# kkaitlyn111/cs336-a2-systems

Measured on AMD Instinct MI355X. Metric: tokens/sec/node GPT-2-XL bf16 DDP, higher is better.
Workload: dtype bf16; 1 GPU; global_batch=102, per_gpu_batch=102, seq_len=512, parallelism=dp1, ddp=none, optimizer=fused HIP AdamW (fp32 master weights), overlapped with backward, attention=HIP FlashAttention-2 (causal), hip_graph=False, gemm_selection=per-problem fastest of hipblaslt default / autotuned lt_gemm / cs336 MFMA GEMM

## Files before the change

### csrc/gemm/gemm8.h

```cpp
#pragma once

#include <hip/hip_runtime.h>
#include <stdint.h>

namespace cs336 {
namespace gemm8 {

struct Args {
  const uint16_t* a;
  const uint16_t* b;
  uint16_t* c;
  uint16_t* h;
  const uint16_t* y;
  int64_t lda, ldb, ldc, ldh, ldy;
  int M, N, K;
  int half;
  const float* rcos;
  const float* rsin;
  const int64_t* rpos;
  int rseq, rope_cols, rdh;
  uint64_t* stamps = nullptr;
};
int pick_fn(int N, int epi, int half);
bool set_stamp_buffer(uint64_t* buf, int64_t blocks);
bool launch(const Args& p, int epi, int fn, hipStream_t s);

struct WArgs {
  const uint16_t* a;
  const uint16_t* b;
  float* c;
  int64_t lda, ldb, ldc, slab_stride;
  int64_t a_elems, b_elems;
  int M, N, K;
  int splits;
  int trans_out, accumulate;
  uint64_t* stamps = nullptr;
  int64_t stamp_rows = 0;
};
bool launch_w(const WArgs& p, int fn, hipStream_t s);

}
}
```

### csrc/gemm/gemm8.hip

```cpp
#include "cs336/kernels.h"
#include "gemm8.h"

namespace cs336 {
namespace gemm8 {


namespace {

typedef __attribute__((ext_vector_type(8))) __bf16 bf16x8;
typedef __attribute__((ext_vector_type(4))) float f32x4;
typedef __attribute__((ext_vector_type(4))) unsigned int v4u32;
typedef __attribute__((address_space(3))) void* lds_ptr_t;

constexpr int BM = 256, BK = 64, NT = 512;
constexpr int kGroupM = 8;

__device__ __forceinline__ int xcd_remap(int bid, int total) {
  const int xcd = bid & 7, q = total >> 3, r = total & 7;
  const int base = xcd < r ? xcd * (q + 1) : r * (q + 1) + (xcd - r) * q;
  return base + (bid >> 3);
}

__device__ __forceinline__ void sbarrier() {
  __builtin_amdgcn_sched_barrier(0);
  asm volatile("s_barrier" ::: "memory");
  __builtin_amdgcn_sched_barrier(0);
}
__device__ __forceinline__ void lgkm0() { asm volatile("s_waitcnt lgkmcnt(0)" ::: "memory"); }
template <int N>
__device__ __forceinline__ void vmcnt() {
  asm volatile("s_waitcnt vmcnt(%0)" ::"n"(N) : "memory");
}

__device__ __forceinline__ float sigmoid_f(float a) { return __builtin_amdgcn_rcpf(1.f + __expf(-a)); }

template <int FN>
struct Geo {
  static constexpr int BN = 64 * FN;
  static constexpr int WTN = 16 * FN;
  static constexpr int FB0 = (FN + 1) / 2;
  static constexpr int B0C = 16 * FB0;
  static constexpr int A_BYTES = BM * 128;
  static constexpr int B_BYTES = BN * 128;
  static constexpr int STAGE = A_BYTES + B_BYTES;
  static constexpr int G_A0 = 16 / 8;
  static constexpr int G_B0 = (4 * B0C / 8) / 8;
  static constexpr int G_B1 = (4 * (WTN - B0C) / 8) / 8;
  static constexpr int G_A1 = 16 / 8;
  static constexpr int G_P1 = G_A0 + G_B0, G_P2 = G_B1, G_P3 = G_A1;
  static constexpr int G_ALL = G_P1 + G_P2 + G_P3;
  static_assert((4 * B0C / 8) % 8 == 0 && (4 * (WTN - B0C) / 8) % 8 == 0, "B granules must split over 8 waves");
};

template <int FN, int EPI, int TAIL>
__global__ __launch_bounds__(NT, 2) void gemm8_kernel(const Args p) {
  static_assert(!TAIL || EPI == 0, "tails: plain C = A·Bᵀ only");
  constexpr bool NTAIL = TAIL & 1, KTAIL = TAIL & 2;
  using G = Geo<FN>;
  constexpr int BN = G::BN, WTN = G::WTN, FB0 = G::FB0, B0C = G::B0C, STAGE = G::STAGE;
  __shared__ __attribute__((aligned(1024))) char smem[2 * STAGE > BM * BN * 2 ? 2 * STAGE : BM * BN * 2];

  const int tid = threadIdx.x, lane = tid & 63;
  const int wave = __builtin_amdgcn_readfirstlane(tid >> 6);
  const int wr = wave >> 2, wc = wave & 3;
#ifdef CS336_G8_STAMP
  const uint64_t st_t0 = __builtin_amdgcn_s_memtime(), st_r0 = __builtin_amdgcn_s_memrealtime();
  uint64_t st_t1 = 0, st_t2 = 0;
#endif

  const int tiles_n = NTAIL ? (p.N + BN - 1) / BN : p.N / BN;
  const int tiles_m = p.M / BM;
  const int bid = xcd_remap(blockIdx.x, gridDim.x);
  const int per_group = kGroupM * tiles_n;
  const int first_m = (bid / per_group) * kGroupM;
  const int gsz = min(tiles_m - first_m, kGroupM);
  const int tm = first_m + (bid % per_group) % gsz, tn = (bid % per_group) / gsz;
  const int m0 = tm * BM;
  const int n0 = tn * (EPI == 1 ? BN / 2 : BN);

  const int nkt = KTAIL ? (p.K + BK - 1) / BK : p.K / BK;
  constexpr uint32_t kOOB = 0x7ffffff0u;
  const __amdgpu_buffer_rsrc_t ra = __builtin_amdgcn_make_buffer_rsrc(
      (void*)(p.a + (int64_t)m0 * p.lda), (short)0, (uint32_t)(((BM - 1) * p.lda + p.K) * 2), 0x00020000);
  const __amdgpu_buffer_rsrc_t rb = __builtin_amdgcn_make_buffer_rsrc(
      (void*)p.b, (short)0, (uint32_t)(((int64_t)(p.N - 1) * p.ldb + p.K) * 2), 0x00020000);
  uint32_t voff[G::G_ALL];
  uint32_t ldso[G::G_ALL];
  {
    int s = 0;
    auto a_gran = [&](int row0) {
      const int r = row0 + (lane >> 3), lc = (lane & 7) ^ ((r >> 1) & 7);
      voff[s] = 2u * (uint32_t)(r * p.lda + lc * 8);
      ldso[s] = (uint32_t)(row0 * 128);
      ++s;
    };
    auto b_gran = [&](int row0) {
      const int r = row0 + (lane >> 3), lc = (lane & 7) ^ ((r >> 1) & 7);
      int grow;
      if constexpr (EPI == 1) grow = r < BN / 2 ? n0 + r : p.half + n0 + (r - BN / 2);
      else grow = n0 + r;
      voff[s] = 2u * (uint32_t)((int64_t)grow * p.ldb + lc * 8);
      ldso[s] = (uint32_t)(G::A_BYTES + row0 * 128);
      ++s;
    };
#pragma unroll
    for (int i = 0; i < G::G_A0; ++i) {
      const int g = wave + 8 * i;
      a_gran(g < 8 ? 8 * g : 128 + 8 * (g - 8));
    }
#pragma unroll
    for (int i = 0; i < G::G_B0; ++i) {
      const int g = wave + 8 * i, per = B0C / 8;
      b_gran((g / per) * WTN + (g % per) * 8);
    }
#pragma unroll
    for (int i = 0; i < G::G_B1; ++i) {
      const int g = wave + 8 * i, per = (WTN - B0C) / 8;
      b_gran((g / per) * WTN + B0C + (g % per) * 8);
    }
#pragma unroll
    for (int i = 0; i < G::G_A1; ++i) {
      const int g = wave + 8 * i;
      a_gran(g < 8 ? 64 + 8 * g : 192 + 8 * (g - 8));
    }
  }
  auto glds = [&](const __amdgpu_buffer_rsrc_t& rs, uint32_t vo, uint32_t so, uint32_t lds_off) {
    __builtin_amdgcn_raw_ptr_buffer_load_lds(rs, (lds_ptr_t)(smem + lds_off), 16, vo, so, 0, 0);
  };
  auto gran_row = [&](int i) -> int {
    if (i < G::G_A0) {
      const int g = wave + 8 * i;
      return g < 8 ? 8 * g : 128 + 8 * (g - 8);
    } else if (i < G::G_P1) {
      const int g = wave + 8 * (i - G::G_A0), per = B0C / 8;
      return (g / per) * WTN + (g % per) * 8;
    } else if (i < G::G_P1 + G::G_P2) {
      const int g = wave + 8 * (i - G::G_P1), per = (WTN - B0C) / 8;
      return (g / per) * WTN + B0C + (g % per) * 8;
    }
    const int g = wave + 8 * (i - G::G_P1 - G::G_P2);
    return g < 8 ? 64 + 8 * g : 192 + 8 * (g - 8);
  };
  auto issue_v = [&](int part, int kt, int st, bool masked) {
    const uint32_t so = (uint32_t)kt * (BK * 2), base = (uint32_t)(st * STAGE);
    auto vo = [&](int i) -> uint32_t {
      if (!masked) return voff[i];
      const int ln = __lane_id(), r = gran_row(i) + (ln >> 3), lc = (ln & 7) ^ ((r >> 1) & 7);
      return kt * BK + lc * 8 >= p.K ? kOOB : voff[i];
    };
    if (part == 0 || part == 1) {
#pragma unroll
      for (int i = 0; i < G::G_A0; ++i) glds(ra, vo(i), so, base + ldso[i]);
#pragma unroll
      for (int i = G::G_A0; i < G::G_P1; ++i) glds(rb, vo(i), so, base + ldso[i]);
    }
    if (part == 0 || part == 2) {
#pragma unroll
      for (int i = G::G_P1; i < G::G_P1 + G::G_P2; ++i) glds(rb, vo(i), so, base + ldso[i]);
    }
    if (part == 0 || part == 3) {
#pragma unroll
      for (int i = G::G_P1 + G::G_P2; i < G::G_ALL; ++i) glds(ra, vo(i), so, base + ldso[i]);
    }
  };
  auto issue = [&](int part, int kt, int st) {
    if (KTAIL && kt == nkt - 1) issue_v(part, kt, st, true);
    else issue_v(part, kt, st, false);
  };

  const int x = (lane & 15) >> 1, q4 = lane >> 4;
  const uint32_t lo0 = (uint32_t)((lane & 15) * 128 + ((q4 ^ x) * 16));
  const uint32_t lo1 = (uint32_t)((lane & 15) * 128 + (((4 + q4) ^ x) * 16));
  auto frag = [&](uint32_t img_off, int row0, int ks) -> bf16x8 {
    const char* ptr = smem + img_off + row0 * 128 + (ks ? lo1 : lo0);
    return __builtin_bit_cast(bf16x8, *reinterpret_cast<const uint4*>(ptr));
  };

  f32x4 acc[8][FN];
#pragma unroll
  for (int i = 0; i < 8; ++i)
#pragma unroll
    for (int j = 0; j < FN; ++j) acc[i][j] = f32x4{0.f, 0.f, 0.f, 0.f};

  bf16x8 fa[4][2], fb0[FB0][2], fb1[FN - FB0 > 0 ? FN - FB0 : 1][2];
  const int arow = wr * 128, bcol = wc * WTN;

  auto mma = [&](int i0, const bf16x8 (&a)[4][2], auto& bq, int j0, int nj) {
    __builtin_amdgcn_s_setprio(1);
#pragma unroll
    for (int ks = 0; ks < 2; ++ks)
#pragma unroll
      for (int i = 0; i < 4; ++i)
#pragma unroll
        for (int j = 0; j < nj; ++j)
          acc[i0 + i][j0 + j] = __builtin_amdgcn_mfma_f32_16x16x32_bf16(bq[j][ks], a[i][ks], acc[i0 + i][j0 + j], 0, 0, 0);
    __builtin_amdgcn_s_setprio(0);
  };

  issue(0, 0, 0);
  if (nkt > 1) {
    issue(0, 1, 1);
    vmcnt<G::G_ALL>();
  } else {
    vmcnt<0>();
  }
  sbarrier();
#ifdef CS336_G8_STAMP
  st_t1 = __builtin_amdgcn_s_memtime();
#endif
  if (wr == 1) sbarrier();

  for (int t = 0; t < nkt; ++t) {
    const uint32_t st = (uint32_t)((t & 1) * STAGE);
    const bool pre = t + 2 < nkt;
#pragma unroll
    for (int i = 0; i < 4; ++i)
#pragma unroll
      for (int ks = 0; ks < 2; ++ks) fa[i][ks] = frag(st, arow + 16 * i, ks);
#pragma unroll
    for (int j = 0; j < FB0; ++j)
#pragma unroll
      for (int ks = 0; ks < 2; ++ks) fb0[j][ks] = frag(st + G::A_BYTES, bcol + 16 * j, ks);
    lgkm0();
    sbarrier();
    mma(0, fa, fb0, 0, FB0);
    sbarrier();
    if constexpr (FN - FB0 > 0) {
#pragma unroll
      for (int j = 0; j < FN - FB0; ++j)
#pragma unroll
        for (int ks = 0; ks < 2; ++ks) fb1[j][ks] = frag(st + G::A_BYTES, bcol + B0C + 16 * j, ks);
    }
    if (pre) issue(1, t + 2, t & 1);
    lgkm0();
    sbarrier();
    if constexpr (FN - FB0 > 0) mma(0, fa, fb1, FB0, FN - FB0);
    sbarrier();
#pragma unroll
    for (int i = 0; i < 4; ++i)
#pragma unroll
      for (int ks = 0; ks < 2; ++ks) fa[i][ks] = frag(st, arow + 64 + 16 * i, ks);
    if (pre) issue(2, t + 2, t & 1);
    lgkm0();
    sbarrier();
    if constexpr (FN - FB0 > 0) mma(4, fa, fb1, FB0, FN - FB0);
    sbarrier();
    if (t + 1 < nkt) {
      if (pre) vmcnt<G::G_P1 + G::G_P2>();
      else vmcnt<0>();
    }
    if (pre) issue(3, t + 2, t & 1);
    sbarrier();
    mma(4, fa, fb0, 0, FB0);
    sbarrier();
  }
  if (wr == 0) sbarrier();
  lgkm0();
  sbarrier();
#ifdef CS336_G8_STAMP
  st_t2 = __builtin_amdgcn_s_memtime();
#endif

  constexpr int ST_AUX = EPI == 0 ? 0 : 2, LD_AUX = 2;
  const int m_l = lane & 15, n_l = 4 * (lane >> 4);
  if constexpr (EPI != 3) {
    constexpr int RB = BN * 2, CH = BN / 8;
    auto img = [&](int row, int ch) -> uint32_t {
      const int x = FN == 5 ? ((row >> 1) & 7) : (row & 15);
      return (uint32_t)(row * RB + ((ch ^ x) << 4));
    };
#pragma unroll
    for (int i = 0; i < 8; ++i)
#pragma unroll
      for (int j = 0; j < FN; ++j) {
        const f32x4 v = acc[i][j];
        const int row = arow + 16 * i + m_l, col = bcol + 16 * j + n_l;
        const uint32_t lo = (uint32_t)f32_to_bf16(v[0]) | ((uint32_t)f32_to_bf16(v[1]) << 16);
        const uint32_t hi = (uint32_t)f32_to_bf16(v[2]) | ((uint32_t)f32_to_bf16(v[3]) << 16);
        *reinterpret_cast<uint2*>(smem + img(row, col >> 3) + ((col >> 2) & 1) * 8) = make_uint2(lo, hi);
      }
    const __amdgpu_buffer_rsrc_t rc = __builtin_amdgcn_make_buffer_rsrc(
        (void*)(p.c + (int64_t)m0 * p.ldc), (short)0, 0x7fffffffu, 0x00020000);
    if constexpr (EPI == 2) {
      constexpr int PT = BM * CH / NT;
      static_assert(BM * CH % NT == 0, "chunks must split over the workgroup");
      const __amdgpu_buffer_rsrc_t ry = __builtin_amdgcn_make_buffer_rsrc(
          (void*)(p.y + (int64_t)m0 * p.ldy), (short)0, 0x7fffffffu, 0x00020000);
      uint4 av[PT], bv[PT];
#pragma unroll
      for (int i = 0; i < PT; ++i) {
        const int q = tid + NT * i, row = q / CH, ch = q % CH;
        const uint32_t off = 2u * (uint32_t)(row * p.ldy + n0 + 8 * ch);
        av[i] = __builtin_bit_cast(uint4, __builtin_amdgcn_raw_buffer_load_b128(ry, off, 0, LD_AUX));
        bv[i] = __builtin_bit_cast(uint4, __builtin_amdgcn_raw_buffer_load_b128(ry, off + 2u * (uint32_t)p.half, 0, LD_AUX));
      }
      lgkm0();
      sbarrier();
#pragma unroll
      for (int i = 0; i < PT; ++i) {
        const int q = tid + NT * i, row = q / CH, ch = q % CH;
        const uint4 dv = *reinterpret_cast<const uint4*>(smem + img(row, ch));
        const bf16_t* de = reinterpret_cast<const bf16_t*>(&dv);
        const bf16_t* ae = reinterpret_cast<const bf16_t*>(&av[i]);
        const bf16_t* be = reinterpret_cast<const bf16_t*>(&bv[i]);
        uint4 dav, dbv;
        bf16_t* da = reinterpret_cast<bf16_t*>(&dav);
        bf16_t* db = reinterpret_cast<bf16_t*>(&dbv);
#pragma unroll
        for (int e = 0; e < 8; ++e) {
          const float a = bf16_to_f32(ae[e]), b = bf16_to_f32(be[e]), dh = bf16_to_f32(de[e]);
          const float sg = sigmoid_f(a), gb = dh * sg;
          da[e] = f32_to_bf16(gb * b * (1.f + a * (1.f - sg)));
          db[e] = f32_to_bf16(gb * a);
        }
        const uint32_t off = 2u * (uint32_t)(row * p.ldc + n0 + 8 * ch);
        __builtin_amdgcn_raw_buffer_store_b128(__builtin_bit_cast(v4u32, dav), rc, off, 0, ST_AUX);
        __builtin_amdgcn_raw_buffer_store_b128(__builtin_bit_cast(v4u32, dbv), rc, off + 2u * (uint32_t)p.half, 0, ST_AUX);
      }
    } else if constexpr (EPI == 1) {
      constexpr int HU = CH / 2, PT = BM * HU / NT;
      static_assert(BM * HU % NT == 0, "pairs must split over the workgroup");
      const __amdgpu_buffer_rsrc_t rh = __builtin_amdgcn_make_buffer_rsrc(
          (void*)(p.h + (int64_t)m0 * p.ldh), (short)0, 0x7fffffffu, 0x00020000);
      lgkm0();
      sbarrier();
#pragma unroll
      for (int i = 0; i < PT; ++i) {
        const int q = tid + NT * i, row = q / HU, u = q % HU;
        const uint4 va = *reinterpret_cast<const uint4*>(smem + img(row, u));
        const uint4 vb = *reinterpret_cast<const uint4*>(smem + img(row, u + HU));
        const uint32_t off = 2u * (uint32_t)(row * p.ldc + n0 + 8 * u);
        __builtin_amdgcn_raw_buffer_store_b128(__builtin_bit_cast(v4u32, va), rc, off, 0, ST_AUX);
        __builtin_amdgcn_raw_buffer_store_b128(__builtin_bit_cast(v4u32, vb), rc, off + 2u * (uint32_t)p.half, 0, ST_AUX);
        const bf16_t* ae = reinterpret_cast<const bf16_t*>(&va);
        const bf16_t* be = reinterpret_cast<const bf16_t*>(&vb);
        uint4 hv;
        bf16_t* he = reinterpret_cast<bf16_t*>(&hv);
#pragma unroll
        for (int e = 0; e < 8; ++e) {
          const float a = bf16_to_f32(ae[e]);
          he[e] = f32_to_bf16(a * sigmoid_f(a) * bf16_to_f32(be[e]));
        }
        __builtin_amdgcn_raw_buffer_store_b128(__builtin_bit_cast(v4u32, hv), rh, 2u * (uint32_t)(row * p.ldh + n0 + 8 * u), 0, ST_AUX);
      }
    } else {
      constexpr int PT = BM * CH / NT;
      lgkm0();
      sbarrier();
#pragma unroll
      for (int i = 0; i < PT; ++i) {
        const int q = tid + NT * i, row = q / CH, ch = q % CH;
        const uint4 v = *reinterpret_cast<const uint4*>(smem + img(row, ch));
        const int col = n0 + 8 * ch;
        if (!NTAIL || col < p.N)
          __builtin_amdgcn_raw_buffer_store_b128(__builtin_bit_cast(v4u32, v), rc, 2u * (uint32_t)(row * p.ldc + col), 0, ST_AUX);
      }
    }
  } else {
    constexpr int CPR = WTN / 8;
    constexpr int PR = 32, UNITS = PR * CPR, PER = UNITS / 64;
    static_assert(UNITS % 64 == 0, "epilogue units must fill the wave");
    char* scr = smem + wave * (PR * WTN * 2);
    constexpr int TOFF = 8 * PR * WTN * 2;
    const int np = p.rdh >> 1;
    const bool rot = n0 < p.rope_cols;
    static_assert(TOFF + 2 * 256 * 48 * 4 <= 2 * STAGE, "cos/sin table of d_head <= 96 behind the scratch");
    if (rot) {
      constexpr int MAXQ = 6;
      float* tc = reinterpret_cast<float*>(smem + TOFF);
      float* ts = tc + 256 * np;
      const int r = tid >> 1, q4n = np >> 2, hq = (q4n + 1) >> 1;
      const int qb = (tid & 1) * hq;
      const int row = m0 + r;
      const int64_t pos = p.rpos ? p.rpos[row] : (int64_t)(row % p.rseq);
      float4 cb[MAXQ], sb[MAXQ];
#pragma unroll
      for (int q = 0; q < MAXQ; ++q) {
        const int i4 = min(qb + q, q4n - 1);
        cb[q] = *reinterpret_cast<const float4*>(p.rcos + pos * np + 4 * i4);
        sb[q] = *reinterpret_cast<const float4*>(p.rsin + pos * np + 4 * i4);
      }
#pragma unroll
      for (int q = 0; q < MAXQ; ++q) {
        const int i4 = min(qb + q, q4n - 1);
        *reinterpret_cast<float4*>(tc + r * np + 4 * i4) = cb[q];
        *reinterpret_cast<float4*>(ts + r * np + 4 * i4) = sb[q];
      }
      __syncthreads();
    }
#pragma unroll
    for (int piece = 0; piece < 128 / PR; ++piece) {
#pragma unroll
      for (int ib = 0; ib < PR / 16; ++ib)
#pragma unroll
        for (int j = 0; j < FN; ++j) {
          const f32x4 v = acc[piece * (PR / 16) + ib][j];
          const uint32_t lo = (uint32_t)f32_to_bf16(v[0]) | ((uint32_t)f32_to_bf16(v[1]) << 16);
          const uint32_t hi = (uint32_t)f32_to_bf16(v[2]) | ((uint32_t)f32_to_bf16(v[3]) << 16);
          *reinterpret_cast<uint2*>(scr + ((16 * ib + m_l) * WTN + 16 * j + n_l) * 2) = make_uint2(lo, hi);
        }
      __builtin_amdgcn_wave_barrier();
#pragma unroll
      for (int u = 0; u < PER; ++u) {
        const int q = lane + 64 * u, rr = q / CPR, cc = q % CPR;
        const uint4 v = *reinterpret_cast<const uint4*>(scr + (rr * WTN + cc * 8) * 2);
        const int64_t row = (int64_t)m0 + arow + PR * piece + rr;
        const int col = n0 + bcol + cc * 8;
        uint4 o = v;
        if (rot) {
          const int i0 = (col % p.rdh) >> 1, tr = arow + PR * piece + rr;
          const float* tc = reinterpret_cast<const float*>(smem + TOFF);
          const float4 c4 = *reinterpret_cast<const float4*>(tc + tr * np + i0);
          const float4 s4 = *reinterpret_cast<const float4*>(tc + 256 * np + tr * np + i0);
          const float cv[4] = {c4.x, c4.y, c4.z, c4.w}, sv[4] = {s4.x, s4.y, s4.z, s4.w};
          const uint32_t w[4] = {v.x, v.y, v.z, v.w};
          uint32_t r[4];
#pragma unroll
          for (int e = 0; e < 4; ++e) {
            const float x0 = bf16_to_f32((bf16_t)(w[e] & 0xffff)), x1 = bf16_to_f32((bf16_t)(w[e] >> 16));
            r[e] = (uint32_t)f32_to_bf16(cv[e] * x0 - sv[e] * x1) |
                   ((uint32_t)f32_to_bf16(sv[e] * x0 + cv[e] * x1) << 16);
          }
          o = make_uint4(r[0], r[1], r[2], r[3]);
        }
        *reinterpret_cast<uint4*>(p.c + row * p.ldc + col) = o;
      }
      lgkm0();
      __builtin_amdgcn_wave_barrier();
    }
  }
#ifdef CS336_G8_STAMP
  vmcnt<0>();
  __syncthreads();
  if (tid == 0 && p.stamps) {
    uint32_t hw, xcc;
    asm volatile("s_getreg_b32 %0, hwreg(HW_REG_HW_ID)" : "=s"(hw));
    asm volatile("s_getreg_b32 %0, hwreg(HW_REG_XCC_ID)" : "=s"(xcc));
    uint64_t* o = p.stamps + 8 * (int64_t)blockIdx.x;
    const uint64_t t3 = __builtin_amdgcn_s_memtime(), r3 = __builtin_amdgcn_s_memrealtime();
    o[0] = st_t0; o[1] = st_t1; o[2] = st_t2; o[3] = t3; o[4] = st_r0; o[5] = r3; o[6] = hw; o[7] = xcc;
  }
#endif
}

uint64_t* g_stamps = nullptr;
int64_t g_stamp_blocks = 0;

template <int FN, int EPI>
void launch_t(const Args& p_in, hipStream_t s) {
  Args p = p_in;
  constexpr int BN = 64 * FN;
  const int tail = EPI == 0 ? (p.N % BN != 0 ? 1 : 0) | (p.K % BK != 0 ? 2 : 0) : 0;
  const int tiles_n = (tail & 1) ? (p.N + BN - 1) / BN : p.N / BN;
  const dim3 grid((unsigned)((p.M / BM) * tiles_n)), block(NT);
  if (g_stamps && (int64_t)grid.x <= g_stamp_blocks) p.stamps = g_stamps;
  if constexpr (EPI == 0) {
    if (tail == 1) {
      hipLaunchKernelGGL((gemm8_kernel<FN, 0, 1>), grid, block, 0, s, p);
      return;
    }
    if (tail == 2) {
      hipLaunchKernelGGL((gemm8_kernel<FN, 0, 2>), grid, block, 0, s, p);
      return;
    }
    if (tail == 3) {
      hipLaunchKernelGGL((gemm8_kernel<FN, 0, 3>), grid, block, 0, s, p);
      return;
    }
  }
  hipLaunchKernelGGL((gemm8_kernel<FN, EPI, 0>), grid, block, 0, s, p);
}

}

bool set_stamp_buffer(uint64_t* buf, int64_t blocks) {
  g_stamps = blocks > 0 ? buf : nullptr;
  g_stamp_blocks = blocks > 0 ? blocks : 0;
#ifdef CS336_G8_STAMP
  return true;
#else
  return false;
#endif
}

int pick_fn(int N, int epi, int half) {
  if (epi == 1) {
    if (half % 160 == 0) return 5;
    if (half % 128 == 0) return 4;
    return 0;
  }
  if (N % 320 == 0) return 5;
  if (N % 256 == 0) return 4;
  if (epi == 0 && N % 8 == 0 && N > 0) {
    const int p5 = (N + 319) / 320 * 320, p4 = (N + 255) / 256 * 256;
    return p4 < p5 ? 4 : 5;
  }
  return 0;
}

bool launch(const Args& p, int epi, int fn, hipStream_t s) {
  if (p.M % BM || p.M <= 0 || p.N <= 0 || p.K <= 0) return false;
  if (epi == 0 ? (p.K % 8 || p.N % 8) : (p.K % BK != 0)) return false;
  if (fn == 0) fn = pick_fn(p.N, epi, p.half);
  if (fn != 4 && fn != 5) return false;
  if (epi != 0 && p.N % (64 * fn)) return false;
  const int64_t lim = (int64_t)0x7fffffff - (1 << 20);
  if (((int64_t)(BM - 1) * p.lda + p.K) * 2 >= lim || ((int64_t)(p.N - 1) * p.ldb + p.K) * 2 >= lim) return false;
  if (epi != 3) {
    const int64_t c_cols = epi == 2 ? (int64_t)p.N + p.half : (int64_t)p.N;
    if (((int64_t)(BM - 1) * p.ldc + c_cols) * 2 >= lim) return false;
    if (epi == 1 && ((int64_t)(BM - 1) * p.ldh + p.half) * 2 >= lim) return false;
    if (epi == 2 && ((int64_t)(BM - 1) * p.ldy + p.N + p.half) * 2 >= lim) return false;
  }
#define CS336_G8(F, E)        \
  do {                        \
    launch_t<F, E>(p, s);     \
    return true;              \
  } while (0)
  if (fn == 5) {
    if (epi == 0) CS336_G8(5, 0);
    if (epi == 1) CS336_G8(5, 1);
    if (epi == 2) CS336_G8(5, 2);
    if (epi == 3) CS336_G8(5, 3);
  } else {
    if (epi == 0) CS336_G8(4, 0);
    if (epi == 1) CS336_G8(4, 1);
    if (epi == 2) CS336_G8(4, 2);
    if (epi == 3) CS336_G8(4, 3);
  }
#undef CS336_G8
  return false;
}

}
}
```

Measured before the change: 92300 tokens/s.

## Restructure GEMM8 main loop into two phases with all B fragments loaded once

The main loop of the MFMA GEMM goes from four barrier-separated MMA phases to two. All B fragments are now loaded once per k-tile, and the global-to-LDS prefetch is regrouped into two parts (B+A0, then A1), with the second part issued for tile t+1 at the start of the next iteration. Precomputed LDS addresses are advanced by a stage delta instead of being recomputed. The intent is fewer barriers and LDS waits per k-tile, at the cost of more fragment registers and a shorter prefetch distance for part of the A tile. The change also adds optional per-phase timing instrumentation, compiled only when the stamp macro is 2 or higher.

```diff
diff --git a/csrc/gemm/gemm8.h b/csrc/gemm/gemm8.h
--- a/csrc/gemm/gemm8.h
+++ b/csrc/gemm/gemm8.h
@@ -20,6 +20,7 @@
   const int64_t* rpos;
   int rseq, rope_cols, rdh;
   uint64_t* stamps = nullptr;
+  int64_t stamp_rows = 0;
 };
 int pick_fn(int N, int epi, int half);
 bool set_stamp_buffer(uint64_t* buf, int64_t blocks);
diff --git a/csrc/gemm/gemm8.hip b/csrc/gemm/gemm8.hip
--- a/csrc/gemm/gemm8.hip
+++ b/csrc/gemm/gemm8.hip
@@ -49,6 +49,7 @@
   static constexpr int G_A1 = 16 / 8;
   static constexpr int G_P1 = G_A0 + G_B0, G_P2 = G_B1, G_P3 = G_A1;
   static constexpr int G_ALL = G_P1 + G_P2 + G_P3;
+  static constexpr int G_X = G_P1 + G_P2, G_Y = G_P3;
   static_assert((4 * B0C / 8) % 8 == 0 && (4 * (WTN - B0C) / 8) % 8 == 0, "B granules must split over 8 waves");
 };
 
@@ -57,7 +58,7 @@
   static_assert(!TAIL || EPI == 0, "tails: plain C = A·Bᵀ only");
   constexpr bool NTAIL = TAIL & 1, KTAIL = TAIL & 2;
   using G = Geo<FN>;
-  constexpr int BN = G::BN, WTN = G::WTN, FB0 = G::FB0, B0C = G::B0C, STAGE = G::STAGE;
+  constexpr int BN = G::BN, WTN = G::WTN, B0C = G::B0C, STAGE = G::STAGE;
   __shared__ __attribute__((aligned(1024))) char smem[2 * STAGE > BM * BN * 2 ? 2 * STAGE : BM * BN * 2];
 
   const int tid = threadIdx.x, lane = tid & 63;
@@ -152,15 +153,11 @@
 #pragma unroll
       for (int i = 0; i < G::G_A0; ++i) glds(ra, vo(i), so, base + ldso[i]);
 #pragma unroll
-      for (int i = G::G_A0; i < G::G_P1; ++i) glds(rb, vo(i), so, base + ldso[i]);
+      for (int i = G::G_A0; i < G::G_X; ++i) glds(rb, vo(i), so, base + ldso[i]);
     }
     if (part == 0 || part == 2) {
 #pragma unroll
-      for (int i = G::G_P1; i < G::G_P1 + G::G_P2; ++i) glds(rb, vo(i), so, base + ldso[i]);
-    }
-    if (part == 0 || part == 3) {
-#pragma unroll
-      for (int i = G::G_P1 + G::G_P2; i < G::G_ALL; ++i) glds(ra, vo(i), so, base + ldso[i]);
+      for (int i = G::G_X; i < G::G_ALL; ++i) glds(ra, vo(i), so, base + ldso[i]);
     }
   };
   auto issue = [&](int part, int kt, int st) {
@@ -169,11 +166,26 @@
   };
 
   const int x = (lane & 15) >> 1, q4 = lane >> 4;
-  const uint32_t lo0 = (uint32_t)((lane & 15) * 128 + ((q4 ^ x) * 16));
-  const uint32_t lo1 = (uint32_t)((lane & 15) * 128 + (((4 + q4) ^ x) * 16));
-  auto frag = [&](uint32_t img_off, int row0, int ks) -> bf16x8 {
-    const char* ptr = smem + img_off + row0 * 128 + (ks ? lo1 : lo0);
-    return __builtin_bit_cast(bf16x8, *reinterpret_cast<const uint4*>(ptr));
+  const int arow = wr * 128, bcol = wc * WTN;
+  uint32_t ada[2], adb[2];
+#pragma unroll
+  for (int ks = 0; ks < 2; ++ks) {
+    const uint32_t lo = (uint32_t)((lane & 15) * 128 + (((4 * ks + q4) ^ x) * 16));
+    ada[ks] = lo + (uint32_t)(arow * 128);
+    adb[ks] = lo + (uint32_t)(G::A_BYTES + bcol * 128);
+  }
+  auto frag = [&](uint32_t addr, int row0) -> bf16x8 {
+    return __builtin_bit_cast(bf16x8, *reinterpret_cast<const uint4*>(smem + addr + row0 * 128));
+  };
+  auto next_stage = [&](int t) {
+    const uint32_t d = (t & 1) ? (uint32_t)(-STAGE) : (uint32_t)STAGE;
+#pragma unroll
+    for (int ks = 0; ks < 2; ++ks) {
+      ada[ks] += d;
+      asm volatile("" : "+v"(ada[ks]));
+      adb[ks] += d;
+      asm volatile("" : "+v"(adb[ks]));
+    }
   };
 
   f32x4 acc[8][FN];
@@ -182,20 +194,41 @@
 #pragma unroll
     for (int j = 0; j < FN; ++j) acc[i][j] = f32x4{0.f, 0.f, 0.f, 0.f};
 
-  bf16x8 fa[4][2], fb0[FB0][2], fb1[FN - FB0 > 0 ? FN - FB0 : 1][2];
-  const int arow = wr * 128, bcol = wc * WTN;
-
-  auto mma = [&](int i0, const bf16x8 (&a)[4][2], auto& bq, int j0, int nj) {
+  bf16x8 fa[4][2], fb[FN][2];
+
+  auto mma = [&](int i0) {
     __builtin_amdgcn_s_setprio(1);
 #pragma unroll
     for (int ks = 0; ks < 2; ++ks)
 #pragma unroll
       for (int i = 0; i < 4; ++i)
 #pragma unroll
-        for (int j = 0; j < nj; ++j)
-          acc[i0 + i][j0 + j] = __builtin_amdgcn_mfma_f32_16x16x32_bf16(bq[j][ks], a[i][ks], acc[i0 + i][j0 + j], 0, 0, 0);
+        for (int j = 0; j < FN; ++j)
+          acc[i0 + i][j] = __builtin_amdgcn_mfma_f32_16x16x32_bf16(fb[j][ks], fa[i][ks], acc[i0 + i][j], 0, 0, 0);
     __builtin_amdgcn_s_setprio(0);
   };
+
+#if CS336_G8_STAMP >= 2
+  constexpr int kStampTiles = 4, kPhases = 2;
+  const bool st_ph = p.stamps && p.stamp_rows >= 5 * (int64_t)gridDim.x;
+  const int s_lo = nkt > kStampTiles ? (nkt - kStampTiles) / 2 : 0;
+  uint32_t s_work[4] = {0, 0, 0, 0}, s_wait[4] = {0, 0, 0, 0}, s_mma[4] = {0, 0, 0, 0}, s_cnt = 0;
+  auto stamp = [&]() -> uint32_t {
+    uint64_t v;
+    __builtin_amdgcn_sched_barrier(0);
+    asm volatile("s_memtime %0\n\ts_waitcnt lgkmcnt(0)" : "=s"(v)::"memory");
+    __builtin_amdgcn_sched_barrier(0);
+    return (uint32_t)v;
+  };
+#define CS336_G8_PSTAMP(I) \
+  do {                     \
+    if (samp) ts_[I] = stamp(); \
+  } while (0)
+#else
+#define CS336_G8_PSTAMP(I) \
+  do {                     \
+  } while (0)
+#endif
 
   issue(0, 0, 0);
   if (nkt > 1) {
@@ -211,54 +244,78 @@
   if (wr == 1) sbarrier();
 
   for (int t = 0; t < nkt; ++t) {
-    const uint32_t st = (uint32_t)((t & 1) * STAGE);
-    const bool pre = t + 2 < nkt;
+    const bool more1 = t + 1 < nkt, more2 = t + 2 < nkt;
+#if CS336_G8_STAMP >= 2
+    const bool samp = st_ph && t >= s_lo && t < s_lo + kStampTiles;
+    uint32_t ts_[3 * kPhases + 1] = {};
+#endif
+    CS336_G8_PSTAMP(0);
+    if (t > 0 && more1) issue(2, t + 1, (t + 1) & 1);
 #pragma unroll
     for (int i = 0; i < 4; ++i)
 #pragma unroll
-      for (int ks = 0; ks < 2; ++ks) fa[i][ks] = frag(st, arow + 16 * i, ks);
-#pragma unroll
-    for (int j = 0; j < FB0; ++j)
-#pragma unroll
-      for (int ks = 0; ks < 2; ++ks) fb0[j][ks] = frag(st + G::A_BYTES, bcol + 16 * j, ks);
+      for (int ks = 0; ks < 2; ++ks) fa[i][ks] = frag(ada[ks], 16 * i);
+#pragma unroll
+    for (int j = 0; j < FN; ++j)
+#pragma unroll
+      for (int ks = 0; ks < 2; ++ks) fb[j][ks] = frag(adb[ks], 16 * j);
+    if (more1) vmcnt<G::G_ALL>();
+    else vmcnt<0>();
     lgkm0();
+    CS336_G8_PSTAMP(1);
     sbarrier();
-    mma(0, fa, fb0, 0, FB0);
+    CS336_G8_PSTAMP(2);
+    mma(0);
     sbarrier();
-    if constexpr (FN - FB0 > 0) {
-#pragma unroll
-      for (int j = 0; j < FN - FB0; ++j)
-#pragma unroll
-        for (int ks = 0; ks < 2; ++ks) fb1[j][ks] = frag(st + G::A_BYTES, bcol + B0C + 16 * j, ks);
-    }
-    if (pre) issue(1, t + 2, t & 1);
+    CS336_G8_PSTAMP(3);
+    if (more2) issue(1, t + 2, t & 1);
+#pragma unroll
+    for (int i = 0; i < 4; ++i)
+#pragma unroll
+      for (int ks = 0; ks < 2; ++ks) fa[i][ks] = frag(ada[ks], 64 + 16 * i);
+    if (more2) vmcnt<G::G_ALL>();
+    else if (more1) vmcnt<G::G_Y>();
     lgkm0();
+    CS336_G8_PSTAMP(4);
     sbarrier();
-    if constexpr (FN - FB0 > 0) mma(0, fa, fb1, FB0, FN - FB0);
+    CS336_G8_PSTAMP(5);
+    mma(4);
+    next_stage(t);
     sbarrier();
-#pragma unroll
-    for (int i = 0; i < 4; ++i)
-#pragma unroll
-      for (int ks = 0; ks < 2; ++ks) fa[i][ks] = frag(st, arow + 64 + 16 * i, ks);
-    if (pre) issue(2, t + 2, t & 1);
-    lgkm0();
-    sbarrier();
-    if constexpr (FN - FB0 > 0) mma(4, fa, fb1, FB0, FN - FB0);
-    sbarrier();
-    if (t + 1 < nkt) {
-      if (pre) vmcnt<G::G_P1 + G::G_P2>();
-      else vmcnt<0>();
-    }
-    if (pre) issue(3, t + 2, t & 1);
-    sbarrier();
-    mma(4, fa, fb0, 0, FB0);
-    sbarrier();
-  }
+    CS336_G8_PSTAMP(6);
+#if CS336_G8_STAMP >= 2
+    if (samp) {
+#pragma unroll
+      for (int ph = 0; ph < kPhases; ++ph) {
+        s_work[ph] += ts_[3 * ph + 1] - ts_[3 * ph];
+        s_wait[ph] += ts_[3 * ph + 2] - ts_[3 * ph + 1];
+        s_mma[ph] += ts_[3 * ph + 3] - ts_[3 * ph + 2];
+      }
+      ++s_cnt;
+    }
+#endif
+  }
+#undef CS336_G8_PSTAMP
   if (wr == 0) sbarrier();
   lgkm0();
   sbarrier();
 #ifdef CS336_G8_STAMP
   st_t2 = __builtin_amdgcn_s_memtime();
+#endif
+#if CS336_G8_STAMP >= 2
+  if (st_ph && lane == 0 && wc == 0) {
+    uint32_t hw, xcc;
+    asm volatile("s_getreg_b32 %0, hwreg(HW_REG_HW_ID)" : "=s"(hw));
+    asm volatile("s_getreg_b32 %0, hwreg(HW_REG_XCC_ID)" : "=s"(xcc));
+    uint64_t* o = p.stamps + 8 * (int64_t)gridDim.x + 32 * (int64_t)blockIdx.x + 16 * wr;
+#pragma unroll
+    for (int ph = 0; ph < kPhases; ++ph) {
+      o[ph] = s_work[ph];
+      o[4 + ph] = s_wait[ph];
+      o[8 + ph] = s_mma[ph];
+    }
+    o[12] = s_cnt; o[13] = (uint64_t)nkt; o[14] = hw; o[15] = xcc;
+  }
 #endif
 
   constexpr int ST_AUX = EPI == 0 ? 0 : 2, LD_AUX = 2;
@@ -453,7 +510,10 @@
   const int tail = EPI == 0 ? (p.N % BN != 0 ? 1 : 0) | (p.K % BK != 0 ? 2 : 0) : 0;
   const int tiles_n = (tail & 1) ? (p.N + BN - 1) / BN : p.N / BN;
   const dim3 grid((unsigned)((p.M / BM) * tiles_n)), block(NT);
-  if (g_stamps && (int64_t)grid.x <= g_stamp_blocks) p.stamps = g_stamps;
+  if (g_stamps && (int64_t)grid.x <= g_stamp_blocks) {
+    p.stamps = g_stamps;
+    p.stamp_rows = g_stamp_blocks;
+  }
   if constexpr (EPI == 0) {
     if (tail == 1) {
       hipLaunchKernelGGL((gemm8_kernel<FN, 0, 1>), grid, block, 0, s, p);
```

New measurement: 93490 tokens/s (median of 6 runs). 1.01x the previous value.
